# NVIDIA/k8s-operator-libs

Hardware: NVIDIA H100
Metric: node state-transitions/sec (higher is better)
Workload: dtype u8/i32

## Files before the change

k8s-operator-libs_b200/csrc/ust_api.cu:

```cuda
#include <cuda_runtime.h>
#include <dlfcn.h>
#include <nccl.h>

#include <cstdarg>
#include <cstdio>
#include <cstdlib>
#include <cstring>
#include <algorithm>
#include <chrono>
#include <mutex>
#include <string>
#include <vector>

#include "ust_dev.h"

namespace {

thread_local std::string g_create_error;

struct NcclApi {
  void* lib = nullptr;
  ncclResult_t (*GetUniqueId)(ncclUniqueId*) = nullptr;
  ncclResult_t (*CommInitRank)(ncclComm_t*, int, ncclUniqueId, int) = nullptr;
  ncclResult_t (*AllReduce)(const void*, void*, size_t, ncclDataType_t, ncclRedOp_t, ncclComm_t, cudaStream_t) = nullptr;
// ... 323 lines not shown
  if (active && !P.requestor && !h->no_hint) {
    unsigned long long sig = 1469598103934665603ull;
    const long long parts[6] = {n, tn, policy->max_parallel_upgrades, policy->max_unavailable_kind, policy->max_unavailable_value, h->world * 64 + h->rank};
    for (long long v : parts) { sig ^= (unsigned long long)v; sig *= 1099511628211ull; }
    P.spec_sig = sig ? sig : 1;
  }
  P.tile_nodes = tn;
  P.n_tiles = tiles;
  P.tile_begin = 0;
  P.tile_end = tiles;
  P.static_rounds = pick_static_rounds(h, tiles, grid);
  P.publish = 1;
  P.stamps = (h->stamps && grid <= UST_MAX_CTAS) ? 1 : 0;
  P.evict_first_inputs = (size_t)n * 13u <= h->l2_bytes ? 1 : 0;
  for (auto& b : h->s_candtile) {
    if ((size_t)tiles + 1 > b.cap && h->last_stream) cudaStreamSynchronize(h->last_stream);
    cudaError_t ce = b.reserve((size_t)tiles + 1);
    if (ce != cudaSuccess) return h->fail(UST_ERR_CUDA, "cudaMalloc failed: %s", cudaGetErrorString(ce));
  }
  if (P.fused_exchange) P.epoch = ++h->epoch;
  P.parity = (int)(h->call_seq++ & 1u);
  P.cand_tile = h->s_candtile[P.parity].p;
  h->prev_n = -1;
  h->ws_dirty = true;
  *out = P;
  *grid_out = grid;
  return UST_OK;
}

static int launch_verify(ust_handle* h, UstParams& P, cudaStream_t st, bool pdl) {
  if (P.split) {
    ncclResult_t r = g_nccl.AllReduce(h->xchg_dev, h->xchg_dev, UST_V_LEN, ncclInt64, ncclSum, h->comm, st);
    if (r != ncclSuccess) return h->fail(UST_ERR_COMM, "ncclAllReduce failed: %s", g_nccl.GetErrorString ? g_nccl.GetErrorString(r) : "?");
  }
  int e = ust_launch_verify(P, h->num_sms, st, (pdl && !P.split) ? 1 : 0);
  if (e) return h->fail(UST_ERR_CUDA, "verification kernel launch failed: %s", cudaGetErrorString((cudaError_t)e));
  h->launches += 1;
  h->verify_ctas += (unsigned long long)h->num_sms;
  return UST_OK;
}

static int check_pod_offsets_host(ust_handle* h, int64_t n, const int32_t* pod_off, int64_t n_pods, int32_t* lens = nullptr) {
  if (n == 0) return UST_OK;
  if (pod_off[0] != 0) return h->fail(UST_ERR_INVALID_ARGUMENT, "pod_off[0] must be 0");
  for (int64_t i = 0; i < n; i++) {
    if (pod_off[i + 1] < pod_off[i]) return h->fail(UST_ERR_INVALID_ARGUMENT, "pod_off must not decrease (node %lld)", (long long)i);
    if (lens) lens[i] = pod_off[i + 1] - pod_off[i];
  }
  if ((int64_t)pod_off[n] != n_pods) return h->fail(UST_ERR_INVALID_ARGUMENT, "pod_off[n_nodes] must equal n_pods");
  return UST_OK;
}

static int apply_device(ust_handle* h, const ust_policy* policy, int64_t n, const uint8_t* state, const uint32_t* flags,
                        const int32_t* pod_rev, const int32_t* ds_idx, int32_t n_ds, const int32_t* ds_rev,
                        const int32_t* pod_off, const uint16_t* pod_flags, int64_t n_pods, uint8_t* next_state,
                        uint16_t* actions, uint8_t* outcome, ust_counters* out_dev, cudaStream_t st) {
  const bool chain = h->chain_entry;
  h->chain_entry = false;
  if (!chain) h->prev_n = -1;
  if (n < 0) return h->fail(UST_ERR_NIL_STATE, "currentState should not be empty");
  if (n > 0 && (!state || !flags || !pod_rev || !ds_idx || !next_state || !actions))
    return h->fail(UST_ERR_NIL_STATE, "currentState should not be empty");
  if (n_ds < 0 || (n_ds > 0 && !ds_rev)) return h->fail(UST_ERR_INVALID_ARGUMENT, "bad DaemonSet table");
  if (n >= (1LL << 40)) return h->fail(UST_ERR_INVALID_ARGUMENT, "too many nodes");
  const void* ptrs[] = {state, flags, pod_rev, ds_idx, next_state, actions, outcome};
  const char* names[] = {"state", "flags", "pod_rev", "ds_idx", "next_state", "actions", "actuator_outcome"};
  for (int i = 0; i < 7; i++)
    if (ptrs[i]) { int rc = check_aligned(h, ptrs[i], names[i]); if (rc) return rc; }
  if (pod_off && pod_flags) { int rc = check_aligned(h, pod_flags, "pod_flags"); if (rc) return rc; }
  UST_CUDA(h, cudaSetDevice(h->device));
  const bool prev_known = h->prev_n >= 0;
  UstParams P;
  int grid = 0;
  int rc = begin_call(h, policy, n, state, flags, pod_rev, ds_idx, n_ds, ds_rev, pod_off, pod_flags, next_state, actions,
                      outcome, out_dev, st, &P, &grid);
  if (rc) return rc;

  if (P.eval_pods) {
    UST_CUDA(h, h->s_podsum.reserve((size_t)n + 16));
    P.podsum = h->s_podsum.p;
    P.evict_first_inputs = 1;
    const int validation = !ust_validation_mode(policy) ? 0 : (policy->validation_enabled ? 2 : 1);
    int e = ust_launch_pod_summary(n, P.active, P.hot, P.pod_off, P.pod_flags, n_pods, P.podlut, P.podsum, P.flags, validation,
                                   &P.ws->errinv[P.parity], h->num_sms * 6, st);
    if (e) return h->fail(UST_ERR_CUDA, "pod-summary kernel launch failed: %s", cudaGetErrorString((cudaError_t)e));
    h->launches += 1;
  }
  ust_handle::Span in[4] = {{(const char*)state, (size_t)n}, {(const char*)flags, (size_t)n * 4}, {(const char*)pod_rev, (size_t)n * 4},
                            {(const char*)ds_idx, (size_t)n * 4}};
  ust_handle::Span outs[3] = {{(const char*)next_state, (size_t)n}, {(const char*)actions, (size_t)n * 2},
                             {(const char*)outcome, outcome ? (size_t)n : 0}};
  auto overlaps = [](const ust_handle::Span& a, const ust_handle::Span& b) {
    return a.len && b.len && a.p < b.p + b.len && b.p < a.p + a.len;
  };
  bool relaxed = chain && h->pdl && h->overlap_calls && st == h->stream && prev_known && !P.eval_pods && !P.split;
  for (int i = 0; relaxed && i < 3; i++) {
    for (int j = 0; j < 3; j++) relaxed = relaxed && !overlaps(outs[i], h->prev_out[j]);
    for (int j = 0; j < 4; j++) relaxed = relaxed && !overlaps(outs[i], h->prev_in[j]);
  }
  for (int i = 0; relaxed && i < 4; i++)
    for (int j = 0; j < 3; j++) relaxed = relaxed && !overlaps(in[i], h->prev_out[j]);
  P.relaxed = relaxed ? 1 : 0;
  h->relaxed_calls += relaxed ? 1 : 0;
  if (relaxed) {
    P.static_rounds = P.n_tiles / grid + 3;
    P.verify_before = h->verify_ctas - (unsigned long long)h->num_sms;
  }
  int e = ust_launch_stream(P, grid, st, h->pdl ? 1 : 0);
  if (e) return h->fail(UST_ERR_CUDA, "streaming kernel launch failed: %s", cudaGetErrorString((cudaError_t)e));
  h->launches += 1;
  rc = launch_verify(h, P, st, h->pdl);
  if (rc) return rc;
  h->ws_dirty = false;
  if (chain && st == h->stream && !P.eval_pods) {
    for (int i = 0; i < 4; i++) h->prev_in[i] = in[i];
    for (int i = 0; i < 3; i++) h->prev_out[i] = outs[i];
    h->prev_n = n;
  }
  return UST_OK;
}

static int finish_with_counters(ust_handle* h, cudaStream_t st, ust_counters* out, bool fetched = false) {
  if (!fetched) UST_CUDA(h, cudaMemcpyAsync(h->counters_host, h->counters_dev, sizeof(ust_counters), cudaMemcpyDeviceToHost, st));
  cudaError_t e = cudaStreamSynchronize(st);
  if (e != cudaSuccess) {
    h->ws_dirty = true;
    return h->fail(UST_ERR_CUDA, "kernel execution failed: %s", cudaGetErrorString(e));
  }
  if (out) *out = *h->counters_host;
  const int code = (int)h->counters_host->error_code;
  if (code != UST_OK) {
    switch (code) {
      case UST_ERR_REVISION_HASH:
        return h->fail(code, "failed to get daemonset template/pod revision hash (node index %lld, pass %lld)",
                       (long long)h->counters_host->error_index, (long long)h->counters_host->error_pass);
      case UST_ERR_MAX_UNAVAILABLE: return h->fail(code, "failed to compute maxUnavailable from the current total nodes");
      case UST_ERR_POD_DELETION_SPEC: return h->fail(code, "pod deletion spec should not be empty");
      case UST_ERR_DS_UNSCHEDULED: return h->fail(code, "driver DaemonSet should not have Unscheduled pods");
      case UST_ERR_COMM: return h->fail(code, "multi-GPU exchange timed out: a peer rank did not take part in the call");
      default: return h->fail(code, "ApplyState aborted with code %d", code);
    }
  }
  return UST_OK;
}

struct StreamDrain {
  ust_handle* h;
  bool armed = true;
  explicit StreamDrain(ust_handle* hh) : h(hh) {}
  ~StreamDrain() {
    if (!armed) return;
    if (h->stream_h2d) cudaStreamSynchronize(h->stream_h2d);
    if (h->stream) cudaStreamSynchronize(h->stream);
    if (h->stream_d2h) cudaStreamSynchronize(h->stream_d2h);
  }
};

#pragma GCC visibility push(default)

struct HostNodes {
  const uint8_t* state;
  const uint32_t* flags;
  const int32_t* rev;
  const int32_t* ds;
  const uint16_t* rev16;
  const int8_t* ds8;
};
// ... 1363 lines not shown
```

k8s-operator-libs_b200/csrc/ust_dev.h:

```cpp
#pragma once
#include <stdint.h>

#include "../../include/ust.h"
#include "ust_lut.h"

#define UST_THREADS 256
#ifndef UST_VERIFY_THREADS
#define UST_VERIFY_THREADS 384
#endif
#define UST_MAX_CTAS 1024
#define UST_MAX_WORLD 8
#define UST_DS_SMEM_MAX 1024

#ifndef UST_TILE_NODES
#define UST_TILE_NODES 3072
#endif
#ifndef UST_STAGES
#define UST_STAGES 4
#endif
#ifndef UST_CONSUMER_WARPS
#define UST_CONSUMER_WARPS 12
#endif
#define UST_STREAM_THREADS (32 * (1 + UST_CONSUMER_WARPS))
#ifndef UST_STREAM_CTAS_PER_SM
#define UST_STREAM_CTAS_PER_SM 1
#endif
#ifndef UST_STREAM_GRID_PER_SM
#define UST_STREAM_GRID_PER_SM 1
#endif
#define UST_STREAM_MAXREG 64
#ifndef UST_VERIFY_MAXREG
#define UST_VERIFY_MAXREG 80
#endif
#define UST_VERIFY_SMEM_MAX 6144

#define UST_V_HIST 0
#define UST_V_UNAVAILABLE 16
#define UST_V_CANDIDATES 17
#define UST_V_RANK_CAND (18)
#define UST_V_RANK_NODES (18 + UST_MAX_WORLD)
#define UST_V_RANK_ERRINV (18 + 2 * UST_MAX_WORLD)
#define UST_V_LEN (18 + 3 * UST_MAX_WORLD)

#define UST_MBOX_WORDS (2 * UST_V_LEN)
struct UstMailbox {
  unsigned long long slot[2][UST_MAX_WORLD][UST_MBOX_WORDS + 12];
};

#define UST_MAX_SEGMENTS 16
struct UstWorkspace {
  unsigned long long acc[2][18];
  unsigned long long errinv[2];
  unsigned int ticket[2][UST_MAX_SEGMENTS];
  int spec_used[2];
  unsigned long long bs_acc[18];
  unsigned int arrive;
  unsigned int comm_timeout;
  long long xsum[2][UST_V_LEN];
  unsigned long long xflag[2];
  unsigned long long hint_sig[2];
  int hint_cut[2];
  unsigned long long verify_done;
  unsigned long long dbg[2][UST_MAX_CTAS][4];
  unsigned int dbg_sm[2][UST_MAX_CTAS];
  unsigned long long dbg2[16];
};

#define UST_KEY(pass, gidx_plus1) ((((unsigned long long)(pass)) << 56) | (unsigned long long)(gidx_plus1))

struct UstParams {
  long long n;
  const uint8_t* hot;
  const uint32_t* flags;
  const int32_t* pod_rev;
  const int32_t* ds_idx;
  const int32_t* ds_rev;
  int n_ds;
  const int32_t* pod_off;
  const uint16_t* pod_flags;
  uint8_t* next;
  uint16_t* actions;
  uint8_t* outcome;
  const uint32_t* lut;
  const uint8_t* podlut;
  uint8_t* podsum;
  UstWorkspace* ws;
  unsigned int* cand_tile;
  long long* xchg;
  ust_counters* out;
  long long max_parallel;
  long long max_unav_value;
  int max_unav_kind;
  int active;
  int requestor;
  int pd_enabled;
  int pd_spec_present;
  int eval_pods;
  int spec_cut_tile;
  unsigned long long spec_sig;
  int rank;
  int world;
  int tile_nodes;
  int n_tiles;
  int tile_begin;
  int tile_end;
  int static_rounds;
  int parity;
  int seg;
  int publish;
  int split;
  int relaxed;
  unsigned long long verify_before;
  int evict_first_inputs;
  int stamps;
  int fused_exchange;
  long long epoch;
  UstMailbox* mbox[UST_MAX_WORLD];
};

int ust_launch_stream(const UstParams& p, int grid, void* stream, int pdl);
int ust_launch_verify(const UstParams& p, int grid, void* stream, int pdl);
int ust_stream_config(int device, int* num_sms, size_t* smem_bytes, int* ctas_per_sm);
int ust_launch_pod_summary(long long n, int active, const uint8_t* hot, const int32_t* pod_off, const uint16_t* pod_flags,
                           long long n_pods, const uint8_t* podlut, uint8_t* podsum, const uint32_t* flags, int validation,
                           unsigned long long* errinv, int grid, void* stream);
int ust_launch_build_state(long long n, const uint8_t* hot, const int32_t* ds_idx, int n_ds, const int32_t* ds_desired,
                           unsigned long long* ds_count, UstWorkspace* ws, ust_counters* out, int grid, void* stream);
#ifdef __CUDACC__
__host__ __device__
#endif
static inline unsigned ust_uid_hash(unsigned long long x, unsigned long long y) {
  unsigned h = (unsigned)x * 0x9E3779B9u + (unsigned)(x >> 32) * 0x85EBCA6Bu + (unsigned)y * 0xC2B2AE35u + (unsigned)(y >> 32) * 0x27D4EB2Fu;
  return h ^ (h >> 15);
}
int ust_launch_build_state_uids(long long n, const uint8_t* hot, const void* owner_uid, int n_ds, const void* ds_tab,
                                const int32_t* ds_tab_idx, int tab_slots, const int32_t* ds_desired, int32_t* ds_idx_out,
                                unsigned long long* ds_count, UstWorkspace* ws, ust_counters* out, int grid, void* stream);
int ust_launch_build_state_delta(long long n, const uint8_t* hot, const void* owner_uid, int n_ds, const void* ds_tab,
                                 const int32_t* ds_tab_idx, int tab_slots, const int32_t* ds_desired, const int32_t* prev,
                                 int32_t* cur, unsigned int* tile_count, unsigned long long* ds_count, UstWorkspace* ws,
                                 ust_counters* out, int grid, void* stream);
int ust_launch_build_state_write(long long n, const int32_t* cur, const int32_t* prev, unsigned int* tile_count, long long* n_out,
                                 long long cap, long long* out_idx, int32_t* out_ds, void* stream);
int ust_build_state_tiles(long long n);
int ust_launch_build_state_reorder(long long n, long long n_runs, const long long* run_off, const long long* run_src,
                                   const uint8_t* ins_hot, const void* ins_uid, const uint8_t* hot, const void* uid,
                                   const int32_t* prev, uint8_t* o_hot, void* o_uid, int32_t* o_prev, void* stream);
int ust_launch_build_state_patch(long long m, const long long* idx, const uint8_t* state, const void* uid, uint8_t* hot_out,
                                 void* uid_out, void* stream);
int ust_launch_patch(long long m, const long long* idx, const uint8_t* state, const uint32_t* flags, const int32_t* pod_rev,
                     const int32_t* ds_idx, uint8_t* hot_out, uint32_t* flags_out, int32_t* rev_out, int32_t* ds_out, void* stream,
                     const long long* start = nullptr, long long* start_out = nullptr);
int ust_launch_clock(long long n, const uint8_t* hot, uint32_t* flags, const long long* start, long long now, long long wait_timeout,
                     int grid, void* stream);
int ust_launch_splice(long long n, long long n_rm, const long long* rm, long long n_ins, const long long* ib, const uint8_t* ins_hot,
                      const uint32_t* ins_flags, const int32_t* ins_rev, const int32_t* ins_ds, const uint8_t* hot, const uint32_t* flags,
                      const int32_t* rev, const int32_t* ds, const uint8_t* next, const uint16_t* act, uint8_t* o_hot, uint32_t* o_flags,
                      int32_t* o_rev, int32_t* o_ds, uint8_t* o_next, uint16_t* o_act, void* stream);
int ust_launch_reorder(long long n, long long n_runs, const long long* run_off, const long long* run_src, const uint8_t* ins_hot,
                       const uint32_t* ins_flags, const int32_t* ins_rev, const int32_t* ins_ds, const uint8_t* hot, const uint32_t* flags,
                       const int32_t* rev, const int32_t* ds, const uint8_t* next, const uint16_t* act, const uint8_t* oc, uint8_t* o_hot,
                       uint32_t* o_flags, int32_t* o_rev, int32_t* o_ds, uint8_t* o_next, uint16_t* o_act, uint8_t* o_oc, void* stream,
                       const long long* ins_start = nullptr, const long long* start = nullptr, long long* o_start = nullptr);
struct UstSimParams {
  int timed;
  long long now, dt;
  long long wait_timeout, job_seconds, validation_seconds, validation_timeout, maintenance_seconds;
};
int ust_launch_feedback(long long n, uint8_t* hot, uint32_t* flags, int32_t* pod_rev, const int32_t* ds_idx, int n_ds,
                        const int32_t* ds_rev, const uint8_t* next, const uint16_t* actions, const uint8_t* outcome,
                        const ust_counters* step, const UstSimParams& sp, int32_t* entered, int32_t* wait_start,
                        int32_t* valid_start, int grid, void* stream);
int ust_launch_sim_init(long long n, const uint32_t* flags, int32_t* entered, int32_t* wait_start, int32_t* valid_start, int grid,
                        void* stream);
int ust_launch_widen(long long n, const uint16_t* rev16, const int8_t* ds8, int32_t* rev_out, int32_t* ds_out, int grid,
                     void* stream);
int ust_launch_diff(long long n, const uint8_t* next, const uint16_t* actions, const uint8_t* outcome, const uint8_t* prev_next,
                    const uint16_t* prev_actions, const uint8_t* prev_outcome, unsigned int* block_count, long long* n_out, long long cap,
                    long long* out_idx, uint8_t* out_next, uint16_t* out_actions, uint8_t* out_outcome, void* stream);
int ust_diff_blocks(long long n);
int ust_launch_pods_scatter(long long n_lists, const long long* node_idx, const int32_t* new_off, const uint16_t* new_flags,
                            const int32_t* off, uint16_t* flags, int grid, void* stream);
int ust_launch_pods_relayout(long long n, long long n_lists, const long long* node_idx, const int32_t* new_off, const int32_t* shift,
                             const int32_t* off, const uint16_t* flags, const uint16_t* new_flags, int new_total, int32_t* runs,
                             int32_t* o_off, uint16_t* o_flags, int grid, void* stream);
int ust_launch_pods_reorder(long long n, long long n_segs, const long long* segs, int32_t* seg_pods, const int32_t* off,
                            const uint16_t* flags, const int32_t* new_off, const uint16_t* new_flags, int new_total, int32_t* o_off,
                            uint16_t* o_flags, int grid, void* stream);
```

k8s-operator-libs_b200/csrc/ust_kernels.cu:

```cuda
#include <climits>

#include "ust_common.cuh"

using namespace ustd;

namespace {

constexpr int kThreads = UST_THREADS;
constexpr int kWarps = kThreads / 32;
constexpr int kVThreads = UST_VERIFY_THREADS;
constexpr int kVWarps = kVThreads / 32;
constexpr int kVStep = kVThreads * 4;
constexpr uint32_t kLutBytes = UST_LUT_WORDS * sizeof(uint32_t);
constexpr int kSimNone = INT32_MIN;
constexpr int kSimLongAgo = -(1 << 30);
constexpr int kDsSmem = 64;

struct __align__(128) Shared {
  uint32_t lut[UST_LUT_ENTRIES];
  uint2 meta[16];
  unsigned long long mbar;
  unsigned long long xflag;
  int dsrev[kDsSmem + 1];
  unsigned int warp_tot[kVWarps];
// ... 266 lines not shown
  if (t == 0) {
    mbar_init(&S.mbar, 1);
    mbar_fence_init();
    mbar_arrive_expect_tx(&S.mbar, kLutBytes);
    bulk_g2s(S.lut, P.lut, kLutBytes, &S.mbar);
  }
  if (P.stamps && t == 0 && (blockIdx.x == 0 || blockIdx.x == gridDim.x - 1)) P.ws->dbg2[blockIdx.x == 0 ? 8 : 9] = now_ns();
  griddep_launch_dependents();
  griddep_wait();
  const bool lead = blockIdx.x == 0;
  if (P.stamps && lead && t == 0) P.ws->dbg2[0] = now_ns();
  bool comm_ok = true;
  if (P.split) {
    if (t < UST_V_LEN) S.D.V[t] = P.xchg[t];
  } else {
    load_local_vector(P, S.D);
    if (t < 32) {
      __syncwarp();
      if (t == 14) fix_excluded_lane(P, S.D);
    }
    if (P.fused_exchange) {
      __syncthreads();
      const int par = (int)(P.epoch & 1);
      const unsigned long long tag = (unsigned long long)(unsigned)P.epoch << 32;
      if (lead) {
        comm_ok = exchange_vector(P, S.D, true);
        if (t < UST_V_LEN) P.ws->xsum[par][t] = S.D.V[t];
        __syncthreads();
        if (t == 0) st_release_gpu(reinterpret_cast<long long*>(&P.ws->xflag[par]), (long long)(tag | (comm_ok ? 1ull : 0ull)));
      } else {
        if (t == 0) {
          const unsigned long long t0 = now_ns();
          unsigned long long v = (unsigned long long)ld_acquire_gpu(reinterpret_cast<const long long*>(&P.ws->xflag[par]));
          while ((v >> 32) != (tag >> 32)) {
            if (now_ns() - t0 > 2 * kCommTimeoutNs) { v = tag; break; }
            __nanosleep(100);
            v = (unsigned long long)ld_acquire_gpu(reinterpret_cast<const long long*>(&P.ws->xflag[par]));
          }
          S.xflag = v;
        }
        __syncthreads();
        comm_ok = (S.xflag & 1ull) != 0;
        if (t < UST_V_LEN) S.D.V[t] = __ldcg(&P.ws->xsum[par][t]);
      }
    }
  }
  if (t == 0) S.D.spec_cut = __ldcg(&P.ws->spec_used[P.parity]);
  __syncthreads();
  if (P.stamps && lead && t == 0) P.ws->dbg2[1] = now_ns();
  decide(P, S.D, lead, !comm_ok);
  if (P.stamps && lead && t == 0) P.ws->dbg2[2] = now_ns();
  const int redo = S.D.redo;
  mbar_wait(&S.mbar, 0);
  if (redo == 0) { verify_cta_done(P); return; }
  if (t == 0) {
    S.redo = redo; S.cut = S.D.cut; S.lo = S.D.lo; S.hi = S.D.hi; S.slots = S.D.slots_left;
    S.abort_key = S.D.abort_key; S.node_offset = S.D.node_offset;
  }
  if (P.n_ds <= kDsSmem)
    for (int i = t; i <= P.n_ds; i += kVThreads) S.dsrev[i] = i < P.n_ds ? __ldg(P.ds_rev + i) : 0;
  __syncthreads();
  int first = S.lo, last = S.hi;
  if (redo == 2) { first = 0; last = P.n_tiles - 1; }
  const int m = last - first + 1;
  const int steps_per_tile = (P.tile_nodes + kVStep - 1) / kVStep;
  if (m >= (int)gridDim.x) {
    const int per = (m + (int)gridDim.x - 1) / (int)gridDim.x;
    const int ta = first + (int)blockIdx.x * per, tb = ta + per < last + 1 ? ta + per : last + 1;
    if (ta < tb) redo_range(P, S, ta, tb);
  } else {
    const int items = m * steps_per_tile;
    for (int it = (int)blockIdx.x; it < items; it += (int)gridDim.x) {
      const int tile = first + it / steps_per_tile, st = it % steps_per_tile;
      redo_steps(P, S, tile, st, st + 1);
      __syncthreads();
    }
  }
  if (P.stamps && lead && t == 0) P.ws->dbg2[3] = now_ns();
  verify_cta_done(P);
}

constexpr int kPodBlock = 4096;
constexpr int kPodChunks = 6;
constexpr int kValWalk = 2;

__device__ __forceinline__ uint32_t validation_summary(const uint16_t* __restrict__ pod_flags, const unsigned char* bytes,
                                                       long long total_bytes, int p0, int p1, uint32_t fl, bool walk) {
  bool not_ready = false, ready_before = false;
  const int len = p1 - p0;
  if (walk && len > 0) {
    const long long c0 = (2LL * p0) & ~15LL;
    const int nchunks = (int)((2LL * p1 - c0 + 15) >> 4);
    if (c0 + 16LL * nchunks <= total_bytes) {
      const uint4* src = reinterpret_cast<const uint4*>(bytes + c0);
      int rel = (int)((c0 >> 1) - p0);
      for (int cb = 0; cb < nchunks && !not_ready; cb += kPodChunks) {
        uint4 x[kPodChunks];
#pragma unroll
        for (int u = 0; u < kPodChunks; u++) x[u] = cb + u < nchunks ? __ldcs(src + cb + u) : make_uint4(0u, 0u, 0u, 0u);
#pragma unroll
        for (int u = 0; u < kPodChunks; u++) {
          const uint32_t wv[4] = {x[u].x, x[u].y, x[u].z, x[u].w};
#pragma unroll
          for (int e = 0; e < 8; e++) {
            const uint32_t f = (e & 1) ? wv[e >> 1] >> 16 : wv[e >> 1];
            if (!not_ready && (f & UST_POD_MATCH_VALIDATION_SELECTOR) && (unsigned)(rel + e) < (unsigned)len) {
              if (f & UST_POD_READY) ready_before = true;
              else not_ready = true;
            }
          }
          rel += 8;
        }
      }
    } else {
      for (int p = p0; p < p1 && !not_ready; p++) {
        const uint32_t f = __ldg(pod_flags + p);
        if (f & UST_POD_MATCH_VALIDATION_SELECTOR) {
          if (f & UST_POD_READY) ready_before = true;
          else not_ready = true;
        }
      }
    }
  }
  return ust_validation_byte(not_ready, ready_before, walk, fl);
}

template <bool VALIDATION>
__global__ void __launch_bounds__(kThreads, 6) ust_pod_summary_kernel(long long n, int active, const uint8_t* __restrict__ hot,
                                                                      const int32_t* __restrict__ pod_off,
                                                                      const uint16_t* __restrict__ pod_flags, long long n_pods,
                                                                      const uint8_t* __restrict__ podlut, uint8_t* __restrict__ podsum,
                                                                      const uint32_t* __restrict__ flags, int validation,
                                                                      unsigned long long* __restrict__ errinv) {
  __shared__ __align__(16) uint8_t lut[256];
  __shared__ __align__(16) uint8_t res[kPodBlock];
  __shared__ unsigned short list[kPodBlock];
  __shared__ int cnt;
  const int t = threadIdx.x, lane = t & 31;
  if (t < 64) reinterpret_cast<uint32_t*>(lut)[t] = __ldg(reinterpret_cast<const uint32_t*>(podlut) + t);
  const unsigned char* bytes = reinterpret_cast<const unsigned char*>(pod_flags);
  const long long total_bytes = 2 * n_pods;
  auto load_hot = [&](long long base) -> uint4 {
    const long long i0 = base + 16 * t;
    uint32_t w[4] = {0x0E0E0E0Eu, 0x0E0E0E0Eu, 0x0E0E0E0Eu, 0x0E0E0E0Eu};
    if (i0 + 16 <= n) return __ldg(reinterpret_cast<const uint4*>(hot + i0));
    for (int k = 0; k < 16; k++)
      if (i0 + k < n) w[k >> 2] = (w[k >> 2] & ~(0xFFu << (8 * (k & 3)))) | ((uint32_t)hot[i0 + k] << (8 * (k & 3)));
    return make_uint4(w[0], w[1], w[2], w[3]);
  };
  for (long long base = (long long)blockIdx.x * kPodBlock; base < n; base += (long long)gridDim.x * kPodBlock) {
    if (t == 0) cnt = 0;
    __syncthreads();
    const long long i0 = base + 16 * t;
    const uint4 hv = load_hot(base);
    const uint32_t w[4] = {hv.x, hv.y, hv.z, hv.w};
    unsigned needbits = 0;
    uint32_t init[4];
#pragma unroll
    for (int k = 0; k < 16; k++) {
      const unsigned s = (w[k >> 2] >> (8 * (k & 3))) & 15u;
      const bool val = VALIDATION && s == UST_STATE_VALIDATION_REQUIRED;
      const bool need = active && ((s >= UST_STATE_WAIT_FOR_JOBS_REQUIRED && s <= UST_STATE_DRAIN_REQUIRED) || val);
      const uint32_t b = need ? (val ? 0xC0u : (((s - UST_STATE_WAIT_FOR_JOBS_REQUIRED) << 6) | (s == UST_STATE_WAIT_FOR_JOBS_REQUIRED ? 0x10u : 0u))) : 0u;
      if ((k & 3) == 0) init[k >> 2] = 0;
      init[k >> 2] |= b << (8 * (k & 3));
      needbits |= (need ? 1u : 0u) << k;
    }
    *reinterpret_cast<uint4*>(res + 16 * t) = make_uint4(init[0], init[1], init[2], init[3]);
    const int mine_cnt = __popc(needbits);
    int incl = mine_cnt;
#pragma unroll
    for (int o = 1; o < 32; o <<= 1) {
      const int v = __shfl_up_sync(kFull, incl, o);
      if (lane >= o) incl += v;
    }
    int wbase = 0;
    if (lane == 31) wbase = atomicAdd(&cnt, incl);
    wbase = __shfl_sync(kFull, wbase, 31);
    int slot = wbase + incl - mine_cnt;
    while (needbits) {
      const int k = __ffs(needbits) - 1;
      needbits &= needbits - 1;
      list[slot++] = (unsigned short)(16 * t + k);
    }
    __syncthreads();
    const int total = cnt;
    for (int q = t; q < total; q += kThreads) {
      const int li = list[q];
      const long long i = base + li;
      const int p0 = __ldg(pod_off + i), p1 = __ldg(pod_off + i + 1);
      const int len = p1 - p0;
      unsigned r = 0;
      const unsigned tag = res[li];
      if (VALIDATION && tag == 0xC0u) {
        const uint32_t v = validation_summary(pod_flags, bytes, total_bytes, p0, p1, __ldg(flags + i), validation == kValWalk);
        if (((v >> UST_VALSUM_OUTCOME_SHIFT) & 7u) == UST_VAL_ERROR) atomicMax(errinv, ~UST_KEY(10, (unsigned long long)i + 1ull));
        res[li] = (uint8_t)v;
        continue;
      }
      const unsigned s = UST_STATE_WAIT_FOR_JOBS_REQUIRED + (tag >> 6);
      const uint32_t sel = s == UST_STATE_WAIT_FOR_JOBS_REQUIRED ? (uint32_t)UST_POD_MATCH_WAIT_SELECTOR
                         : (s == UST_STATE_POD_DELETION_REQUIRED ? (uint32_t)UST_POD_MATCH_DELETION_FILTER : (uint32_t)UST_POD_MATCH_DRAIN_SELECTOR);
      const unsigned sat = s == UST_STATE_WAIT_FOR_JOBS_REQUIRED ? UST_PODSUM_WAIT_RUNNING
                         : (s == UST_STATE_POD_DELETION_REQUIRED ? (UST_PODSUM_TO_DELETE | UST_PODSUM_CANNOT_DELETE) : UST_PODSUM_DRAIN_ERROR);
      const long long c0 = (2LL * p0) & ~15LL;
      const int nchunks = len > 0 ? (int)((2LL * p1 - c0 + 15) >> 4) : 0;
      const bool safe = c0 + 16LL * nchunks <= total_bytes;
      if (safe) {
        const uint4* src = reinterpret_cast<const uint4*>(bytes + c0);
        int rel = (int)((c0 >> 1) - p0);
        for (int cb = 0; cb < nchunks; cb += kPodChunks) {
          uint4 x[kPodChunks];
#pragma unroll
          for (int u = 0; u < kPodChunks; u++) x[u] = cb + u < nchunks ? __ldcs(src + cb + u) : make_uint4(0u, 0u, 0u, 0u);
#pragma unroll
          for (int u = 0; u < kPodChunks; u++) {
            if (cb + u < nchunks && (r & sat) != sat) {
              const uint32_t wv[4] = {x[u].x, x[u].y, x[u].z, x[u].w};
#pragma unroll
              for (int e = 0; e < 8; e++) {
                const uint32_t f = (e & 1) ? wv[e >> 1] >> 16 : wv[e >> 1];
                if ((f & sel) && (unsigned)(rel + e) < (unsigned)len) r |= lut[f & 255u];
              }
            }
            rel += 8;
          }
        }
      } else {
        for (int p = p0; p < p1; p++) {
          const uint32_t f = __ldg(pod_flags + p);
          if (f & sel) r |= lut[f & 255u];
        }
      }
      unsigned ps;
      if (s == UST_STATE_WAIT_FOR_JOBS_REQUIRED) ps = 0x10u | (r & UST_PODSUM_WAIT_RUNNING);
      else if (s == UST_STATE_POD_DELETION_REQUIRED) ps = r & (UST_PODSUM_TO_DELETE | UST_PODSUM_CANNOT_DELETE);
      else ps = r & UST_PODSUM_DRAIN_ERROR;
      res[li] = (uint8_t)ps;
    }
    __syncthreads();
    if (i0 + 16 <= n) {
      *reinterpret_cast<uint4*>(podsum + i0) = *reinterpret_cast<const uint4*>(res + 16 * t);
    } else {
      for (int k = 0; k < 16; k++)
        if (i0 + k < n) podsum[i0 + k] = res[16 * t + k];
    }
  }
}

constexpr int kUidTabSmem = 2048;
constexpr int kBuildU = 4;
constexpr int kBuildSpill = 240;

template <bool UID>
__device__ __forceinline__ bool build_prologue(ulonglong2* tab, int* ord, unsigned int* cnt_ds, unsigned long long* inc,
                                               unsigned int* cnt, int n_ds, const ulonglong2* __restrict__ ds_tab,
                                               const int32_t* __restrict__ ds_tab_idx, int tab_slots) {
  const int t = threadIdx.x;
  const bool in_smem = UID ? tab_slots <= kUidTabSmem : n_ds <= kUidTabSmem / 4;
  if (in_smem) {
    if (UID)
      for (int i = t; i < tab_slots; i += kThreads) { tab[i] = ds_tab[i]; ord[i] = ds_tab_idx[i]; }
    for (int i = t; i < n_ds; i += kThreads) cnt_ds[i] = 0;
  }
  inc[t] = hot_increments(t);
  if (t < 16) cnt[t] = 0;
  return in_smem;
}

__device__ __forceinline__ int build_join(const ulonglong2& u, const ulonglong2* table, const int* order, unsigned slot_mask) {
  int d = -2;
  if ((u.x | u.y) == 0ull) {
    d = -1;
  } else {
    unsigned slot = ust_uid_hash(u.x, u.y) & slot_mask;
    for (;;) {
      const ulonglong2 e = table[slot];
      if (e.x == u.x && e.y == u.y) { d = order[slot]; break; }
      if ((e.x | e.y) == 0ull) break;
      slot = (slot + 1u) & slot_mask;
    }
  }
  return d;
}

__device__ __forceinline__ void build_count(unsigned hb, bool owned, const unsigned long long* inc, uint32_t (&B)[4], uint32_t& lo,
                                            uint32_t& hi, int& pending, long long& excluded) {
  if (owned && (hb & 15u) < 14u) {
    const unsigned long long v = inc[hb];
    lo += (uint32_t)v;
    hi += (uint32_t)(v >> 32);
  } else {
    excluded++;
  }
  if ((++pending & 7) == 0) widen(lo, hi, B);
}

__device__ __forceinline__ void build_count_ds(int d, unsigned long long& dsl, unsigned int* cnt_ds, unsigned long long* ds_count,
                                               int n_ds, bool in_smem) {
  if (n_ds <= 8) {
    if (d >= 0) dsl += 1ull << (8 * d);
  } else {
    const unsigned act = __ballot_sync(kFull, d >= 0);
    if (d >= 0) {
      const unsigned peers = __match_any_sync(act, d);
      if ((threadIdx.x & 31) == __ffs(peers) - 1) {
        if (in_smem) atomicAdd(&cnt_ds[d], (unsigned)__popc(peers));
        else atomicAdd(&ds_count[d], (unsigned long long)__popc(peers));
      }
    }
  }
}

__device__ __forceinline__ void build_spill(uint32_t (&B)[4], uint32_t& lo, uint32_t& hi, int& pending, unsigned long long& dsl,
                                            unsigned int* cnt, unsigned int* cnt_ds) {
  widen(lo, hi, B);
#pragma unroll
  for (int f = 0; f < 16; f++) {
    const unsigned v = field_of(B, f);
    if (v) atomicAdd(&cnt[f], v);
  }
// ... 799 lines not shown
  return m;
}
template <bool OUTCOME>
__global__ void __launch_bounds__(kThreads) ust_diff_count_kernel(long long n, const uint8_t* __restrict__ next, const uint16_t* __restrict__ act,
                                                                  const uint8_t* __restrict__ oc, const uint8_t* __restrict__ pnext,
                                                                  const uint16_t* __restrict__ pact, const uint8_t* __restrict__ poc,
                                                                  unsigned int* __restrict__ block_count) {
  __shared__ unsigned int tot;
  if (threadIdx.x == 0) tot = 0;
  __syncthreads();
  const long long i0 = (long long)blockIdx.x * kDiffBlock + 16 * threadIdx.x;
  const unsigned c = i0 < n ? __popc(diff_mask16<OUTCOME>(next, act, oc, pnext, pact, poc, i0, n)) : 0u;
  cta_sum(c, tot);
  if (threadIdx.x == 0) block_count[blockIdx.x] = tot;
}
__global__ void __launch_bounds__(1024) ust_diff_scan_kernel(int blocks, unsigned int* block_count, long long* n_out) {
  __shared__ unsigned long long part[32];
  __shared__ unsigned long long carry;
  const int t = threadIdx.x;
  if (t == 0) carry = 0;
  __syncthreads();
  for (int b0 = 0; b0 < blocks; b0 += 1024) {
    const int b = b0 + t;
    const unsigned long long v = b < blocks ? block_count[b] : 0ull;
    unsigned long long incl = v;
#pragma unroll
    for (int o = 1; o < 32; o <<= 1) {
      const unsigned long long u = __shfl_up_sync(kFull, incl, o);
      if ((t & 31) >= o) incl += u;
    }
    if ((t & 31) == 31) part[t >> 5] = incl;
    __syncthreads();
    unsigned long long before = carry, tot = 0;
    for (int w = 0; w < 32; w++) { if (w < (t >> 5)) before += part[w]; tot += part[w]; }
    if (b < blocks) block_count[b] = (unsigned int)(before + incl - v);
    __syncthreads();
    if (t == 0) carry += tot;
    __syncthreads();
  }
  if (t == 0) *n_out = (long long)carry;
}
template <bool OUTCOME>
__global__ void __launch_bounds__(kThreads) ust_diff_write_kernel(long long n, const uint8_t* __restrict__ next, const uint16_t* __restrict__ act,
                                                                  const uint8_t* __restrict__ oc, const uint8_t* __restrict__ pnext,
                                                                  const uint16_t* __restrict__ pact, const uint8_t* __restrict__ poc,
                                                                  const unsigned int* __restrict__ block_off, long long cap,
                                                                  long long* __restrict__ out_idx, uint8_t* __restrict__ out_next,
                                                                  uint16_t* __restrict__ out_act, uint8_t* __restrict__ out_oc) {
  const int t = threadIdx.x;
  const long long i0 = (long long)blockIdx.x * kDiffBlock + 16 * t;
  const unsigned m = i0 < n ? diff_mask16<OUTCOME>(next, act, oc, pnext, pact, poc, i0, n) : 0u;
  long long pos = cta_first_pos(__popc(m), block_off);
  unsigned mm = m;
  while (mm) {
    const int k = __ffs(mm) - 1;
    mm &= mm - 1;
    if (pos < cap) {
      out_idx[pos] = i0 + k;
      out_next[pos] = next[i0 + k];
      out_act[pos] = act[i0 + k];
      if constexpr (OUTCOME) out_oc[pos] = oc[i0 + k];
    }
    pos++;
  }
}

}

int ust_launch_verify(const UstParams& p, int grid, void* stream, int pdl) {
  cudaLaunchConfig_t cfg = {};
  cfg.gridDim = dim3((unsigned)grid);
  cfg.blockDim = dim3(kVThreads);
  cfg.dynamicSmemBytes = 0;
  cfg.stream = (cudaStream_t)stream;
  cudaLaunchAttribute attr[1];
  attr[0].id = cudaLaunchAttributeProgrammaticStreamSerialization;
  attr[0].val.programmaticStreamSerializationAllowed = 1;
  cfg.attrs = attr;
  cfg.numAttrs = pdl ? 1 : 0;
  return (int)cudaLaunchKernelEx(&cfg, ust_verify_kernel, p);
}
int ust_launch_pod_summary(long long n, int active, const uint8_t* hot, const int32_t* pod_off, const uint16_t* pod_flags,
                           long long n_pods, const uint8_t* podlut, uint8_t* podsum, const uint32_t* flags, int validation,
                           unsigned long long* errinv, int grid, void* stream) {
  if (n <= 0) return 0;
  const long long blocks = (n + kPodBlock - 1) / kPodBlock;
  if (grid > blocks) grid = (int)blocks;
  if (validation)
    ust_pod_summary_kernel<true><<<grid, kThreads, 0, (cudaStream_t)stream>>>(n, active, hot, pod_off, pod_flags, n_pods, podlut,
                                                                            podsum, flags, validation, errinv);
  else
    ust_pod_summary_kernel<false><<<grid, kThreads, 0, (cudaStream_t)stream>>>(n, active, hot, pod_off, pod_flags, n_pods, podlut,
                                                                             podsum, flags, validation, errinv);
  return (int)cudaGetLastError();
}
int ust_launch_build_state(long long n, const uint8_t* hot, const int32_t* ds_idx, int n_ds, const int32_t* ds_desired,
                           unsigned long long* ds_count, UstWorkspace* ws, ust_counters* out, int grid, void* stream) {
  ust_build_state_uid_kernel<false><<<grid, kThreads, 0, (cudaStream_t)stream>>>(n, hot, nullptr, ds_idx, n_ds, nullptr, nullptr, 8,
                                                                                 nullptr, ds_count, ws);
  ust_build_state_finish_kernel<<<1, 1, 0, (cudaStream_t)stream>>>(n_ds, ds_desired, ds_count, ws, out);
  return (int)cudaGetLastError();
}
int ust_launch_widen(long long n, const uint16_t* rev16, const int8_t* ds8, int32_t* rev_out, int32_t* ds_out, int grid,
                     void* stream) {
  if (n <= 0) return 0;
  const long long want = (n + kThreads - 1) / kThreads;
  ust_widen_kernel<<<(unsigned)(want < grid ? want : grid), kThreads, 0, (cudaStream_t)stream>>>(n, rev16, ds8, rev_out, ds_out);
  return (int)cudaGetLastError();
}
int ust_launch_patch(long long m, const long long* idx, const uint8_t* state, const uint32_t* flags, const int32_t* pod_rev,
                     const int32_t* ds_idx, uint8_t* hot_out, uint32_t* flags_out, int32_t* rev_out, int32_t* ds_out, void* stream,
                     const long long* start, long long* start_out) {
  if (m <= 0) return 0;
  const long long grid = (m + kThreads - 1) / kThreads;
  const unsigned g = (unsigned)(grid > 65535 * 16 ? 65535 * 16 : grid);
  if (start_out)
    ust_patch_kernel<true><<<g, kThreads, 0, (cudaStream_t)stream>>>(m, idx, state, flags, pod_rev, ds_idx, hot_out, flags_out, rev_out,
                                                                    ds_out, start, start_out);
  else
    ust_patch_kernel<false><<<g, kThreads, 0, (cudaStream_t)stream>>>(m, idx, state, flags, pod_rev, ds_idx, hot_out, flags_out, rev_out,
                                                                     ds_out, nullptr, nullptr);
  return (int)cudaGetLastError();
}
int ust_launch_clock(long long n, const uint8_t* hot, uint32_t* flags, const long long* start, long long now, long long wait_timeout,
                     int grid, void* stream) {
  if (n <= 0) return 0;
  const long long want = ((n + 15) / 16 + kThreads - 1) / kThreads;
  ust_clock_kernel<<<(unsigned)(want < grid ? want : grid), kThreads, 0, (cudaStream_t)stream>>>(n, hot, flags, start, now, wait_timeout);
  return (int)cudaGetLastError();
}
int ust_launch_splice(long long n, long long n_rm, const long long* rm, long long n_ins, const long long* ib, const uint8_t* ins_hot,
                      const uint32_t* ins_flags, const int32_t* ins_rev, const int32_t* ins_ds, const uint8_t* hot, const uint32_t* flags,
                      const int32_t* rev, const int32_t* ds, const uint8_t* next, const uint16_t* act, uint8_t* o_hot, uint32_t* o_flags,
                      int32_t* o_rev, int32_t* o_ds, uint8_t* o_next, uint16_t* o_act, void* stream) {
  const long long grid = n / kSpliceTile + 1;
  ust_splice_kernel<<<(unsigned)grid, kThreads, 0, (cudaStream_t)stream>>>(n, n_rm, rm, n_ins, ib, ins_hot, ins_flags, ins_rev, ins_ds, hot,
                                                                           flags, rev, ds, next, act, o_hot, o_flags, o_rev, o_ds, o_next, o_act);
  return (int)cudaGetLastError();
}
int ust_launch_reorder(long long n, long long n_runs, const long long* run_off, const long long* run_src, const uint8_t* ins_hot,
                       const uint32_t* ins_flags, const int32_t* ins_rev, const int32_t* ins_ds, const uint8_t* hot, const uint32_t* flags,
                       const int32_t* rev, const int32_t* ds, const uint8_t* next, const uint16_t* act, const uint8_t* oc, uint8_t* o_hot,
                       uint32_t* o_flags, int32_t* o_rev, int32_t* o_ds, uint8_t* o_next, uint16_t* o_act, uint8_t* o_oc, void* stream,
                       const long long* ins_start, const long long* start, long long* o_start) {
  const long long grid = n > 0 ? (n + kGatherTile - 1) / kGatherTile : 1;
  if (oc && o_start)
    ust_reorder_kernel<true, true><<<(unsigned)grid, kThreads, 0, (cudaStream_t)stream>>>(
        n, n_runs, run_off, run_src, ins_hot, ins_flags, ins_rev, ins_ds, hot, flags, rev, ds, next, act, oc, o_hot, o_flags, o_rev, o_ds,
        o_next, o_act, o_oc, ins_start, start, o_start);
  else if (oc)
    ust_reorder_kernel<true, false><<<(unsigned)grid, kThreads, 0, (cudaStream_t)stream>>>(n, n_runs, run_off, run_src, ins_hot, ins_flags, ins_rev,
                                                                                  ins_ds, hot, flags, rev, ds, next, act, oc, o_hot, o_flags,
                                                                                  o_rev, o_ds, o_next, o_act, o_oc, nullptr, nullptr, nullptr);
  else
    ust_reorder_kernel<false, false><<<(unsigned)grid, kThreads, 0, (cudaStream_t)stream>>>(n, n_runs, run_off, run_src, ins_hot, ins_flags, ins_rev,
                                                                                   ins_ds, hot, flags, rev, ds, next, act, nullptr, o_hot,
                                                                                   o_flags, o_rev, o_ds, o_next, o_act, nullptr, nullptr, nullptr,
                                                                                   nullptr);
  return (int)cudaGetLastError();
}
int ust_launch_pods_scatter(long long n_lists, const long long* node_idx, const int32_t* new_off, const uint16_t* new_flags,
                            const int32_t* off, uint16_t* flags, int grid, void* stream) {
  const long long want = (n_lists + kWarps - 1) / kWarps;
  const int g = want < 1 ? 1 : (want < grid ? (int)want : grid);
  ust_pods_scatter_kernel<<<g, kThreads, 0, (cudaStream_t)stream>>>(n_lists, node_idx, new_off, new_flags, off, flags);
  return (int)cudaGetLastError();
}
int ust_launch_pods_relayout(long long n, long long n_lists, const long long* node_idx, const int32_t* new_off, const int32_t* shift,
                             const int32_t* off, const uint16_t* flags, const uint16_t* new_flags, int new_total, int32_t* runs,
                             int32_t* o_off, uint16_t* o_flags, int grid, void* stream) {
// ... 118 lines not shown
```

Before: 179.3 billion.

## Batch pod-summary node walks to overlap first-chunk loads across nodes

The pod-summary kernel now handles several candidate nodes per thread at once. It issues the first two 16-byte pod-flag loads for every node in the batch before doing any evaluation, which gives more memory-level parallelism for the common case of short pod lists. The remaining chunks are walked per node afterwards. The launch grid now covers every block with no persistent cap, and launch bounds drop to 4 CTAs per SM to leave room for the extra registers. In exchange, register pressure rises, and there is some wasted loading for validation-tagged or satisfied nodes.

New measurement: 179.6 billion, median of 6. Within noise of the previous version (+0.1%).

```diff
diff --git a/k8s-operator-libs_b200/csrc/ust_api.cu b/k8s-operator-libs_b200/csrc/ust_api.cu
--- a/k8s-operator-libs_b200/csrc/ust_api.cu
+++ b/k8s-operator-libs_b200/csrc/ust_api.cu
@@ -429,7 +429,7 @@
     P.evict_first_inputs = 1;
     const int validation = !ust_validation_mode(policy) ? 0 : (policy->validation_enabled ? 2 : 1);
     int e = ust_launch_pod_summary(n, P.active, P.hot, P.pod_off, P.pod_flags, n_pods, P.podlut, P.podsum, P.flags, validation,
-                                   &P.ws->errinv[P.parity], h->num_sms * 6, st);
+                                   &P.ws->errinv[P.parity], st);
     if (e) return h->fail(UST_ERR_CUDA, "pod-summary kernel launch failed: %s", cudaGetErrorString((cudaError_t)e));
     h->launches += 1;
   }
diff --git a/k8s-operator-libs_b200/csrc/ust_dev.h b/k8s-operator-libs_b200/csrc/ust_dev.h
--- a/k8s-operator-libs_b200/csrc/ust_dev.h
+++ b/k8s-operator-libs_b200/csrc/ust_dev.h
@@ -33,6 +33,12 @@
 #define UST_VERIFY_MAXREG 80
 #endif
 #define UST_VERIFY_SMEM_MAX 6144
+#ifndef UST_POD_CTAS_PER_SM
+#define UST_POD_CTAS_PER_SM 4
+#endif
+#ifndef UST_POD_BATCH
+#define UST_POD_BATCH 3
+#endif
 
 #define UST_V_HIST 0
 #define UST_V_UNAVAILABLE 16
@@ -123,7 +129,7 @@
 int ust_stream_config(int device, int* num_sms, size_t* smem_bytes, int* ctas_per_sm);
 int ust_launch_pod_summary(long long n, int active, const uint8_t* hot, const int32_t* pod_off, const uint16_t* pod_flags,
                            long long n_pods, const uint8_t* podlut, uint8_t* podsum, const uint32_t* flags, int validation,
-                           unsigned long long* errinv, int grid, void* stream);
+                           unsigned long long* errinv, void* stream);
 int ust_launch_build_state(long long n, const uint8_t* hot, const int32_t* ds_idx, int n_ds, const int32_t* ds_desired,
                            unsigned long long* ds_count, UstWorkspace* ws, ust_counters* out, int grid, void* stream);
 #ifdef __CUDACC__
diff --git a/k8s-operator-libs_b200/csrc/ust_kernels.cu b/k8s-operator-libs_b200/csrc/ust_kernels.cu
--- a/k8s-operator-libs_b200/csrc/ust_kernels.cu
+++ b/k8s-operator-libs_b200/csrc/ust_kernels.cu
@@ -372,6 +372,7 @@
 
 constexpr int kPodBlock = 4096;
 constexpr int kPodChunks = 6;
+constexpr int kPodBatch = UST_POD_BATCH;
 constexpr int kValWalk = 2;
 
 __device__ __forceinline__ uint32_t validation_summary(const uint16_t* __restrict__ pod_flags, const unsigned char* bytes,
@@ -415,8 +416,36 @@
   return ust_validation_byte(not_ready, ready_before, walk, fl);
 }
 
+__device__ __forceinline__ unsigned pod_chunk_or(const uint4 x, int rel, int len, uint32_t sel, const uint8_t* lut) {
+  const uint32_t wv[4] = {x.x, x.y, x.z, x.w};
+  unsigned r = 0;
+#pragma unroll
+  for (int e = 0; e < 8; e++) {
+    const uint32_t f = (e & 1) ? wv[e >> 1] >> 16 : wv[e >> 1];
+    if ((f & sel) && (unsigned)(rel + e) < (unsigned)len) r |= lut[f & 255u];
+  }
+  return r;
+}
+
+template <typename T>
+__device__ __forceinline__ T pod_batch_pick(const T (&a)[kPodBatch], int b) {
+  T v = a[0];
+#pragma unroll
+  for (int k = 1; k < kPodBatch; k++)
+    if (b == k) v = a[k];
+  return v;
+}
+
+__device__ __forceinline__ void pod_state_masks(unsigned tag, uint32_t* sel, unsigned* sat) {
+  const unsigned s = UST_STATE_WAIT_FOR_JOBS_REQUIRED + (tag >> 6);
+  *sel = s == UST_STATE_WAIT_FOR_JOBS_REQUIRED ? (uint32_t)UST_POD_MATCH_WAIT_SELECTOR
+       : (s == UST_STATE_POD_DELETION_REQUIRED ? (uint32_t)UST_POD_MATCH_DELETION_FILTER : (uint32_t)UST_POD_MATCH_DRAIN_SELECTOR);
+  *sat = s == UST_STATE_WAIT_FOR_JOBS_REQUIRED ? UST_PODSUM_WAIT_RUNNING
+       : (s == UST_STATE_POD_DELETION_REQUIRED ? (UST_PODSUM_TO_DELETE | UST_PODSUM_CANNOT_DELETE) : UST_PODSUM_DRAIN_ERROR);
+}
+
 template <bool VALIDATION>
-__global__ void __launch_bounds__(kThreads, 6) ust_pod_summary_kernel(long long n, int active, const uint8_t* __restrict__ hot,
+__global__ void __launch_bounds__(kThreads, UST_POD_CTAS_PER_SM) ust_pod_summary_kernel(long long n, int active, const uint8_t* __restrict__ hot,
                                                                       const int32_t* __restrict__ pod_off,
                                                                       const uint16_t* __restrict__ pod_flags, long long n_pods,
                                                                       const uint8_t* __restrict__ podlut, uint8_t* __restrict__ podsum,
@@ -475,58 +504,83 @@
     }
     __syncthreads();
     const int total = cnt;
-    for (int q = t; q < total; q += kThreads) {
-      const int li = list[q];
-      const long long i = base + li;
-      const int p0 = __ldg(pod_off + i), p1 = __ldg(pod_off + i + 1);
-      const int len = p1 - p0;
-      unsigned r = 0;
-      const unsigned tag = res[li];
-      if (VALIDATION && tag == 0xC0u) {
-        const uint32_t v = validation_summary(pod_flags, bytes, total_bytes, p0, p1, __ldg(flags + i), validation == kValWalk);
-        if (((v >> UST_VALSUM_OUTCOME_SHIFT) & 7u) == UST_VAL_ERROR) atomicMax(errinv, ~UST_KEY(10, (unsigned long long)i + 1ull));
-        res[li] = (uint8_t)v;
-        continue;
-      }
-      const unsigned s = UST_STATE_WAIT_FOR_JOBS_REQUIRED + (tag >> 6);
-      const uint32_t sel = s == UST_STATE_WAIT_FOR_JOBS_REQUIRED ? (uint32_t)UST_POD_MATCH_WAIT_SELECTOR
-                         : (s == UST_STATE_POD_DELETION_REQUIRED ? (uint32_t)UST_POD_MATCH_DELETION_FILTER : (uint32_t)UST_POD_MATCH_DRAIN_SELECTOR);
-      const unsigned sat = s == UST_STATE_WAIT_FOR_JOBS_REQUIRED ? UST_PODSUM_WAIT_RUNNING
-                         : (s == UST_STATE_POD_DELETION_REQUIRED ? (UST_PODSUM_TO_DELETE | UST_PODSUM_CANNOT_DELETE) : UST_PODSUM_DRAIN_ERROR);
-      const long long c0 = (2LL * p0) & ~15LL;
-      const int nchunks = len > 0 ? (int)((2LL * p1 - c0 + 15) >> 4) : 0;
-      const bool safe = c0 + 16LL * nchunks <= total_bytes;
-      if (safe) {
-        const uint4* src = reinterpret_cast<const uint4*>(bytes + c0);
-        int rel = (int)((c0 >> 1) - p0);
-        for (int cb = 0; cb < nchunks; cb += kPodChunks) {
-          uint4 x[kPodChunks];
-#pragma unroll
-          for (int u = 0; u < kPodChunks; u++) x[u] = cb + u < nchunks ? __ldcs(src + cb + u) : make_uint4(0u, 0u, 0u, 0u);
-#pragma unroll
-          for (int u = 0; u < kPodChunks; u++) {
-            if (cb + u < nchunks && (r & sat) != sat) {
-              const uint32_t wv[4] = {x[u].x, x[u].y, x[u].z, x[u].w};
-#pragma unroll
-              for (int e = 0; e < 8; e++) {
-                const uint32_t f = (e & 1) ? wv[e >> 1] >> 16 : wv[e >> 1];
-                if ((f & sel) && (unsigned)(rel + e) < (unsigned)len) r |= lut[f & 255u];
+    for (int q0 = t; q0 < total; q0 += kPodBatch * kThreads) {
+      int li[kPodBatch], p0[kPodBatch], len[kPodBatch];
+#pragma unroll
+      for (int b = 0; b < kPodBatch; b++) {
+        const int q = q0 + b * kThreads;
+        li[b] = -1;
+        p0[b] = len[b] = 0;
+        if (q < total) {
+          li[b] = list[q];
+          p0[b] = __ldg(pod_off + base + li[b]);
+          len[b] = __ldg(pod_off + base + li[b] + 1) - p0[b];
+        }
+      }
+      unsigned r[kPodBatch];
+      {
+        uint4 x[kPodBatch][2];
+#pragma unroll
+        for (int b = 0; b < kPodBatch; b++) {
+          const long long c0 = (2LL * p0[b]) & ~31LL;
+          const long long end = (2LL * (p0[b] + len[b]) + 15) & ~15LL;
+          const bool walk = li[b] >= 0 && len[b] > 0 && end <= total_bytes && !(VALIDATION && res[li[b]] == 0xC0u);
+          const uint4* src = reinterpret_cast<const uint4*>(bytes + c0);
+          x[b][0] = walk ? __ldcs(src) : make_uint4(0u, 0u, 0u, 0u);
+          x[b][1] = walk && end - c0 > 16 ? __ldcs(src + 1) : make_uint4(0u, 0u, 0u, 0u);
+        }
+#pragma unroll
+        for (int b = 0; b < kPodBatch; b++) {
+          uint32_t sel;
+          unsigned sat;
+          pod_state_masks(li[b] >= 0 ? res[li[b]] : 0u, &sel, &sat);
+          const int rel = -(p0[b] & 15);
+          r[b] = pod_chunk_or(x[b][0], rel, len[b], sel, lut) | pod_chunk_or(x[b][1], rel + 8, len[b], sel, lut);
+        }
+      }
+#pragma unroll 1
+      for (int b = 0; b < kPodBatch; b++) {
+        const int l = pod_batch_pick(li, b);
+        if (l < 0) break;
+        const long long i = base + l;
+        const int p = pod_batch_pick(p0, b), n_l = pod_batch_pick(len, b);
+        const unsigned tag = res[l];
+        if (VALIDATION && tag == 0xC0u) {
+          const uint32_t v = validation_summary(pod_flags, bytes, total_bytes, p, p + n_l, __ldg(flags + i), validation == kValWalk);
+          if (((v >> UST_VALSUM_OUTCOME_SHIFT) & 7u) == UST_VAL_ERROR) atomicMax(errinv, ~UST_KEY(10, (unsigned long long)i + 1ull));
+          res[l] = (uint8_t)v;
+          continue;
+        }
+        uint32_t sel;
+        unsigned sat;
+        pod_state_masks(tag, &sel, &sat);
+        unsigned rr = pod_batch_pick(r, b);
+        const long long c0 = (2LL * p) & ~31LL;
+        const int nchunks = n_l > 0 ? (int)((((2LL * (p + n_l) + 15) & ~15LL) - c0) >> 4) : 0;
+        const bool safe = c0 + 16LL * nchunks <= total_bytes;
+        if (safe) {
+          if ((rr & sat) != sat) {
+            const uint4* src = reinterpret_cast<const uint4*>(bytes + c0);
+            int rel = 16 - (p & 15);
+            for (int cb = 2; cb < nchunks; cb += kPodChunks) {
+              uint4 x[kPodChunks];
+#pragma unroll
+              for (int u = 0; u < kPodChunks; u++) x[u] = cb + u < nchunks ? __ldcs(src + cb + u) : make_uint4(0u, 0u, 0u, 0u);
+#pragma unroll
+              for (int u = 0; u < kPodChunks; u++) {
+                if (cb + u < nchunks && (rr & sat) != sat) rr |= pod_chunk_or(x[u], rel, n_l, sel, lut);
+                rel += 8;
               }
             }
-            rel += 8;
+          }
+        } else {
+          for (int k = p; k < p + n_l; k++) {
+            const uint32_t f = __ldg(pod_flags + k);
+            if (f & sel) rr |= lut[f & 255u];
           }
         }
-      } else {
-        for (int p = p0; p < p1; p++) {
-          const uint32_t f = __ldg(pod_flags + p);
-          if (f & sel) r |= lut[f & 255u];
-        }
-      }
-      unsigned ps;
-      if (s == UST_STATE_WAIT_FOR_JOBS_REQUIRED) ps = 0x10u | (r & UST_PODSUM_WAIT_RUNNING);
-      else if (s == UST_STATE_POD_DELETION_REQUIRED) ps = r & (UST_PODSUM_TO_DELETE | UST_PODSUM_CANNOT_DELETE);
-      else ps = r & UST_PODSUM_DRAIN_ERROR;
-      res[li] = (uint8_t)ps;
+        res[l] = (uint8_t)((tag == 0x10u ? 0x10u : 0u) | (rr & sat));
+      }
     }
     __syncthreads();
     if (i0 + 16 <= n) {
@@ -1492,10 +1546,9 @@
 }
 int ust_launch_pod_summary(long long n, int active, const uint8_t* hot, const int32_t* pod_off, const uint16_t* pod_flags,
                            long long n_pods, const uint8_t* podlut, uint8_t* podsum, const uint32_t* flags, int validation,
-                           unsigned long long* errinv, int grid, void* stream) {
+                           unsigned long long* errinv, void* stream) {
   if (n <= 0) return 0;
-  const long long blocks = (n + kPodBlock - 1) / kPodBlock;
-  if (grid > blocks) grid = (int)blocks;
+  const int grid = (int)((n + kPodBlock - 1) / kPodBlock);
   if (validation)
     ust_pod_summary_kernel<true><<<grid, kThreads, 0, (cudaStream_t)stream>>>(n, active, hot, pod_off, pod_flags, n_pods, podlut,
                                                                             podsum, flags, validation, errinv);
```
